# Francis-Fan-create/SCaSML_GP

Hardware: AMD Instinct MI355X
Metric: Euler-Maruyama path-steps/sec + L2 rel-error, Grad_Dependent_Nonlinear d=100 n=3 (higher is better)
Workload: dtype f32

## Files before the change

### include/scasml_hip.h

```cpp
#ifndef SCASML_HIP_H
#define SCASML_HIP_H

#include <stddef.h>
#include <stdint.h>

#ifdef __cplusplus
extern "C" {
#endif

#define SCASML_ABI_VERSION 7
#define SCASML_MAX_LEVEL 5
#define SCASML_MAX_Q 6
#define SCASML_MAX_DIM 252
#define SCASML_GP_TILE 32
#define SCASML_NORMAL_TABLE_ROWS 768

enum { SCASML_ERR_ARG = -1, SCASML_ERR_UNSUPPORTED = -2, SCASML_ERR_HIP = -3 };

enum { SCASML_EQ_GRAD_DEPENDENT_NONLINEAR = 0, SCASML_EQ_CUBIC_REACTION_DIFFUSION = 1, SCASML_EQ_QUADRATIC_GRADIENT_REACTION_DIFFUSION = 2 };

typedef struct {
    int32_t d;
    int32_t eq_id;
    float T;
// ... 138 lines not shown
                              const int32_t *idx_h, int32_t round16, const float *points, int64_t n_inf, int32_t kp, float *grad, void *stream);

int64_t scasml_gp_compat_model_floats(int32_t d, int32_t n_pad);
int scasml_gp_compat_pack_mfma(int32_t d, float a, const float *x_dom, int32_t n_dom, const float *x_bdy, int32_t n_bdy,
                               const double *rv, const int32_t *idx_h, float *model_out, void *stream);
int scasml_gp_eval_compat_sites(int32_t d, float a, float sigma_eq, float mu_eq, int32_t eq_id, const float *model, int32_t n_dom,
                                int32_t n_bdy, const int32_t *idx_h, int32_t round16, float x_bound, const float *points, int64_t n_inf,
                                int64_t rows_per_site, const uint8_t *site_kinds, float *out4, float *lap, void *stream);
int scasml_gp_eval_compat_site_list(int32_t d, float a, float sigma_eq, float mu_eq, int32_t eq_id, const float *model, int32_t n_dom,
                                    int32_t n_bdy, const int32_t *idx_h, int32_t round16, float x_bound, const float *points, int64_t n_inf,
                                    int64_t rows_per_site, const uint8_t *site_kinds, const int32_t *site_order, int32_t n_listed,
                                    float *out4, float *lap, void *stream);

int scasml_gp_cross_rows(int32_t d, double a, const float *x_dom, int32_t n_dom, const float *x_bdy, int32_t n_bdy, const int32_t *idx_h,
                         int32_t round16, int32_t surrogate, int32_t op, const float *x_inf, int64_t n_inf, int64_t ld_inf, double *out,
                         int64_t ld, void *stream);

#define SCASML_DIST_BLOCK 256
int scasml_gp_gram_rows(int32_t d, double a, const float *x_dom, int32_t n_dom, const float *x_bdy, int32_t n_bdy,
                        int64_t row0, int32_t nrows, int64_t ncols, double *out, int64_t ld, void *stream);
int scasml_gp_gram_compat_rows(int32_t d, double a, const float *x_dom, int32_t n_dom, const float *x_bdy, int32_t n_bdy, const int32_t *idx_h,
                               int32_t round16, int64_t row0, int32_t nrows, int64_t ncols, double *out, int64_t ld, void *stream);
int scasml_gemm_nt_sub(double *C, int64_t ldc, int64_t rows, int64_t cols, const double *A, int64_t lda, const double *B,
                       int64_t ldb, int64_t K, int64_t tri_row0, int64_t tri_stride, int64_t tri_col0, void *stream);
int scasml_trsm_right_lt(const double *L, int64_t ldl, int64_t nb, double *X, int64_t ldx, int64_t rows, void *stream);
int scasml_gemv_sub(const double *A, int64_t lda, int64_t rows, int64_t cols, const double *x, double *y, int trans, void *stream);
int64_t scasml_gemv_t_ordered_scratch(int64_t rows, int64_t cols);
int scasml_gemv_t_sub_ordered(const double *A, int64_t lda, int64_t rows, int64_t cols, const double *x, double *y, double *scratch,
                              int64_t scratch_elems, void *stream);
int scasml_gemv_sub_tri(const double *A, int64_t lda, int64_t rows, int64_t cols, const double *x, double *y, int64_t tri_row0, int64_t tri_stride, void *stream);
int scasml_gemv_t_sub_ordered_tri(const double *A, int64_t lda, int64_t rows, int64_t cols, const double *x, double *y, double *scratch,
                                  int64_t scratch_elems, int64_t tri_row0, int64_t tri_stride, void *stream);

#ifdef __cplusplus
}
#endif
#endif
```

### scasml_gp_amd/_build.py

```python
import os
import subprocess
from concurrent.futures import ThreadPoolExecutor

HERE = os.path.dirname(os.path.abspath(__file__))
ROOT = os.path.dirname(HERE)
CSRC = os.path.join(HERE, "csrc")
LIBDIR = os.path.join(HERE, "lib")
LIB = os.path.join(LIBDIR, "libscasml_hip.so")
SOURCES = ["plan_host.cpp", "picard_tree_jax_deep.hip", "picard_tree.hip", "picard_tree_jax.hip", "gp_eval.hip", "gp_eval_bf16.hip", "gp_train.hip", "gp_compat.hip", "gp_eval_compat_mfma.hip", "dist_linalg.hip"]
FLAGS = ["--offload-arch=gfx950", "-O3", "-std=c++17", "-ffp-contract=off", "-fno-slp-vectorize", "-fPIC", "-I" + os.path.join(ROOT, "include")]


def _stale(target, deps):
    if not os.path.exists(target):
        return True
    t = os.path.getmtime(target)
    return any(os.path.getmtime(d) > t for d in deps)


def build_library(force=False, verbose=False):
    hipcc = os.environ.get("HIPCC", "/opt/rocm/bin/hipcc")
    os.makedirs(LIBDIR, exist_ok=True)
    headers = [os.path.join(CSRC, f) for f in os.listdir(CSRC) if f.endswith(".hpp")]
    headers.append(os.path.join(ROOT, "include", "scasml_hip.h"))
    objs, jobs = [], []
    for src in SOURCES:
        s = os.path.join(CSRC, src)
        o = os.path.join(LIBDIR, os.path.splitext(src)[0] + ".o")
        objs.append(o)
        if force or _stale(o, [s] + headers):
            flags = FLAGS if src.endswith(".hip") else [f for f in FLAGS if not f.startswith("--offload-arch")] + ["-x", "c++"]
            jobs.append([hipcc] + flags + ["-c", s, "-o", o])

    def run(cmd):
        if verbose:
            print(" ".join(cmd), flush=True)
        r = subprocess.run(cmd, capture_output=True, text=True)
        if r.returncode != 0:
            raise RuntimeError("hipcc failed:\n" + " ".join(cmd) + "\n" + r.stdout + r.stderr)

    with ThreadPoolExecutor(max_workers=min(8, os.cpu_count() or 4)) as ex:
        list(ex.map(run, jobs))
# ... 8 lines not shown
```

### scasml_gp_amd/_lib.py

```python
import ctypes as C
import os

MAX_LEVEL = 5
MAX_Q = 6
MAX_DIM = 252
GP_TILE = 32
DIST_BLOCK = 256
ABI_VERSION = 7

MODE_MLP, MODE_GENERATE, MODE_ACCUMULATE = 0, 1, 2
RNG_COMPAT_CRN = 1
RNG_COMPAT_F16 = 2
RNG_JAX_STREAM = 4
EQ_GRAD_DEPENDENT_NONLINEAR = 0
EQ_CUBIC_REACTION_DIFFUSION = 1
EQ_QUADRATIC_GRADIENT_REACTION_DIFFUSION = 2


class Problem(C.Structure):
    _fields_ = [("d", C.c_int32), ("eq_id", C.c_int32), ("T", C.c_float), ("mu", C.c_float),
                ("sigma", C.c_float), ("clip", C.c_float)]


class Rng(C.Structure):
    _fields_ = [("seed", C.c_uint64), ("stream", C.c_uint32), ("root0", C.c_uint32),
                ("rank", C.c_int32), ("world", C.c_int32), ("flags", C.c_uint32), ("reserved", C.c_uint32),
                ("unit_owner", C.c_void_p), ("jax_keys", C.c_void_p)]


class Term(C.Structure):
    _fields_ = [("q", C.c_int32), ("mc", C.c_int32), ("sites_l", C.c_int32), ("sites_lm1", C.c_int32),
                ("dfrac", C.c_float * MAX_Q), ("cfrac", C.c_float * MAX_Q),
                ("wfrac", C.c_float * MAX_Q), ("dplus", C.c_float * MAX_Q)]


class Plan(C.Structure):
    _fields_ = [("variant", C.c_int32), ("n", C.c_int32), ("mg", C.c_int32 * (MAX_LEVEL + 1)),
                ("sites", C.c_int32 * (MAX_LEVEL + 1)), ("term", (Term * MAX_LEVEL) * (MAX_LEVEL + 1))]


class GpModel(C.Structure):
    _fields_ = [("d", C.c_int32), ("n_dom", C.c_int32), ("n_bdy", C.c_int32), ("n_pad", C.c_int32),
                ("kp", C.c_int32), ("split", C.c_int32), ("a", C.c_float), ("sigma_eq", C.c_float),
                ("mu_eq", C.c_float), ("eq_id", C.c_int32),
                ("colloc", C.c_void_p), ("colloc_frag", C.c_void_p), ("colloc_bf16", C.c_void_p), ("colloc_is_f16", C.c_int32),
                ("coef", C.c_void_p), ("x_bound", C.c_float), ("reserved", C.c_int32)]


_STRUCTS = (Problem, Rng, Term, Plan, GpModel)
_LIB = None
LIB_PATH = os.environ.get("SCASML_HIP_LIB") or os.path.join(os.path.dirname(os.path.abspath(__file__)), "lib", "libscasml_hip.so")

SIGNATURES = {
    "scasml_abi_version": (C.c_int, []),
    "scasml_last_error": (C.c_char_p, []),
    "scasml_sizeof": (C.c_size_t, [C.c_int]),
    "scasml_points_per_root": (C.c_int64, [C.POINTER(Plan)]),
    "scasml_point_stride": (C.c_int32, [C.c_int32]),
    "scasml_picard_tree": (C.c_int, [C.POINTER(Problem), C.POINTER(Plan), C.c_int, C.c_void_p, C.c_int64, C.c_int64, Rng,
                                     C.c_void_p, C.c_void_p, C.c_void_p, C.c_void_p, C.c_void_p]),
    "scasml_clip": (C.c_int, [C.c_void_p, C.c_int64, C.c_float, C.c_void_p]),
    "scasml_clip_round16": (C.c_int, [C.c_void_p, C.c_int64, C.c_float, C.c_int32, C.c_void_p]),
    "scasml_debug_normals": (C.c_int, [Rng, C.c_uint32, C.c_int32, C.c_int64, C.c_void_p, C.c_void_p]),
    "scasml_debug_jax_normals": (C.c_int, [C.c_uint32, C.c_uint32, C.c_uint64, C.c_int64, C.c_void_p, C.c_void_p]),
    "scasml_debug_transform": (C.c_int, [C.c_uint32, C.c_int64, C.c_void_p, C.c_void_p]),
    "scasml_normal_table_rows": (C.c_int32, []),
    "scasml_normal_table": (C.c_int, [C.c_void_p, C.c_int32]),
    "scasml_gp_plane_halfwords": (C.c_int64, [C.c_int32, C.c_int32]),
    "scasml_gp_coef_floats": (C.c_int64, [C.c_int32]),
    "scasml_gp_pack": (C.c_int, [C.c_int32, C.c_float, C.c_float, C.c_void_p, C.c_int32, C.c_void_p, C.c_int32, C.c_void_p,
                                 C.c_void_p, C.c_void_p, C.c_void_p, C.c_void_p, C.c_void_p]),
    "scasml_gp_eval": (C.c_int, [C.POINTER(GpModel), C.c_void_p, C.c_int64, C.c_void_p, C.c_void_p, C.c_void_p]),
    "scasml_gp_eval_sites": (C.c_int, [C.POINTER(GpModel), C.c_void_p, C.c_int64, C.c_int64, C.c_void_p, C.c_void_p, C.c_void_p]),
    "scasml_plan_site_kinds": (C.c_int, [C.POINTER(Plan), C.c_int32, C.c_int32, C.c_void_p, C.c_void_p]),
    "scasml_plan_deal_units": (C.c_int32, [C.POINTER(Plan), C.c_int32, C.c_void_p, C.c_void_p, C.c_int32, C.c_void_p]),
    "scasml_tile_order_blocks": (C.c_int64, [C.c_int64, C.c_int64, C.c_int32]),
    "scasml_tile_order": (C.c_int, [C.c_int64, C.c_int64, C.c_int64, C.c_int32, C.POINTER(C.c_int64), C.POINTER(C.c_int64)]),
    "scasml_gp_gradient": (C.c_int, [C.POINTER(GpModel), C.c_void_p, C.c_int64, C.c_void_p, C.c_void_p]),
    "scasml_gp_gram": (C.c_int, [C.c_int32, C.c_double, C.c_void_p, C.c_int32, C.c_void_p, C.c_int32, C.c_void_p, C.c_void_p]),
    "scasml_gp_newton_b": (C.c_int, [C.c_int32, C.c_int32, C.c_double, C.c_double, C.c_void_p, C.c_void_p, C.c_int32, C.c_int32, C.c_void_p, C.c_void_p]),
# ... 8 lines not shown
    "scasml_gp_eval_compat": (C.c_int, [C.c_int32, C.c_double, C.c_double, C.c_double, C.c_int32, C.c_void_p, C.c_int32, C.c_int32, C.c_int64, C.c_void_p,
                                        C.c_void_p, C.c_int32, C.c_void_p, C.c_int64, C.c_int32, C.c_void_p, C.c_void_p, C.c_void_p]),
    "scasml_gp_gradient_compat": (C.c_int, [C.c_int32, C.c_double, C.c_void_p, C.c_int32, C.c_int32, C.c_int64, C.c_void_p, C.c_void_p, C.c_int32,
                                            C.c_void_p, C.c_int64, C.c_int32, C.c_void_p, C.c_void_p]),
    "scasml_gp_compat_model_floats": (C.c_int64, [C.c_int32, C.c_int32]),
    "scasml_gp_compat_pack_mfma": (C.c_int, [C.c_int32, C.c_float, C.c_void_p, C.c_int32, C.c_void_p, C.c_int32, C.c_void_p, C.c_void_p,
                                             C.c_void_p, C.c_void_p]),
    "scasml_gp_eval_compat_sites": (C.c_int, [C.c_int32, C.c_float, C.c_float, C.c_float, C.c_int32, C.c_void_p, C.c_int32, C.c_int32, C.c_void_p,
                                              C.c_int32, C.c_float, C.c_void_p, C.c_int64, C.c_int64, C.c_void_p, C.c_void_p, C.c_void_p, C.c_void_p]),
    "scasml_gp_eval_compat_site_list": (C.c_int, [C.c_int32, C.c_float, C.c_float, C.c_float, C.c_int32, C.c_void_p, C.c_int32, C.c_int32, C.c_void_p,
                                                  C.c_int32, C.c_float, C.c_void_p, C.c_int64, C.c_int64, C.c_void_p, C.c_void_p, C.c_int32, C.c_void_p,
                                                  C.c_void_p, C.c_void_p]),
    "scasml_gp_cross_rows": (C.c_int, [C.c_int32, C.c_double, C.c_void_p, C.c_int32, C.c_void_p, C.c_int32, C.c_void_p, C.c_int32, C.c_int32, C.c_int32,
                                       C.c_void_p, C.c_int64, C.c_int64, C.c_void_p, C.c_int64, C.c_void_p]),
    "scasml_gp_gram_rows": (C.c_int, [C.c_int32, C.c_double, C.c_void_p, C.c_int32, C.c_void_p, C.c_int32, C.c_int64, C.c_int32, C.c_int64,
                                      C.c_void_p, C.c_int64, C.c_void_p]),
    "scasml_gp_gram_compat_rows": (C.c_int, [C.c_int32, C.c_double, C.c_void_p, C.c_int32, C.c_void_p, C.c_int32, C.c_void_p, C.c_int32, C.c_int64,
                                             C.c_int32, C.c_int64, C.c_void_p, C.c_int64, C.c_void_p]),
    "scasml_gemm_nt_sub": (C.c_int, [C.c_void_p, C.c_int64, C.c_int64, C.c_int64, C.c_void_p, C.c_int64, C.c_void_p, C.c_int64, C.c_int64,
                                     C.c_int64, C.c_int64, C.c_int64, C.c_void_p]),
    "scasml_gp_newton_jv": (C.c_int, [C.c_int32, C.c_int32, C.c_double, C.c_double, C.c_void_p, C.c_void_p, C.c_int32, C.c_int32, C.c_void_p, C.c_void_p]),
    "scasml_gp_newton_jtv": (C.c_int, [C.c_int32, C.c_int32, C.c_double, C.c_double, C.c_void_p, C.c_void_p, C.c_void_p, C.c_void_p, C.c_double,
                                       C.c_int32, C.c_int32, C.c_void_p, C.c_void_p]),
    "scasml_trsm_right_lt": (C.c_int, [C.c_void_p, C.c_int64, C.c_int64, C.c_void_p, C.c_int64, C.c_int64, C.c_void_p]),
    "scasml_gemv_sub": (C.c_int, [C.c_void_p, C.c_int64, C.c_int64, C.c_int64, C.c_void_p, C.c_void_p, C.c_int, C.c_void_p]),
    "scasml_gemv_t_ordered_scratch": (C.c_int64, [C.c_int64, C.c_int64]),
    "scasml_gemv_t_sub_ordered": (C.c_int, [C.c_void_p, C.c_int64, C.c_int64, C.c_int64, C.c_void_p, C.c_void_p, C.c_void_p, C.c_int64, C.c_void_p]),
    "scasml_gemv_sub_tri": (C.c_int, [C.c_void_p, C.c_int64, C.c_int64, C.c_int64, C.c_void_p, C.c_void_p, C.c_int64, C.c_int64, C.c_void_p]),
    "scasml_gemv_t_sub_ordered_tri": (C.c_int, [C.c_void_p, C.c_int64, C.c_int64, C.c_int64, C.c_void_p, C.c_void_p, C.c_void_p, C.c_int64, C.c_int64, C.c_int64,
                                                C.c_void_p]),
    "scasml_cholesky": (C.c_int, [C.c_void_p, C.c_int64, C.c_double, C.c_void_p, C.c_void_p]),
    "scasml_cholesky_inverse": (C.c_int, [C.c_void_p, C.c_int64, C.c_void_p, C.c_void_p]),
    "scasml_trsm_lower": (C.c_int, [C.c_void_p, C.c_int64, C.c_void_p, C.c_int64, C.c_int, C.c_void_p]),
}


class ScasmlError(RuntimeError):
    pass


def load():
    global _LIB
    if _LIB is not None:
        return _LIB
    import torch
    if not os.path.exists(LIB_PATH):
        raise ScasmlError(
            "libscasml_hip.so is not built (%s missing). Build it with "
            "`python -c 'import __graft_entry__ as g; g.build()'` or `python -m scasml_gp_amd._build`; "
            "scasml_gp_amd has no CPU fallback." % LIB_PATH)
    lib = C.CDLL(LIB_PATH)
    for name, (res, args) in SIGNATURES.items():
        fn = getattr(lib, name)
        fn.restype, fn.argtypes = res, args
    if lib.scasml_abi_version() != ABI_VERSION:
        raise ScasmlError("libscasml_hip.so ABI %d != binding ABI %d" % (lib.scasml_abi_version(), ABI_VERSION))
    for which, st in enumerate(_STRUCTS):
        if lib.scasml_sizeof(which) != C.sizeof(st):
            raise ScasmlError("struct %s: library says %d bytes, binding %d" % (st.__name__, lib.scasml_sizeof(which), C.sizeof(st)))
    _LIB = lib
    return lib


def check(rc, what):
    if rc != 0:
        raise ScasmlError("%s failed (%d): %s" % (what, rc, load().scasml_last_error().decode()))
# ... 17 lines not shown
```

### scasml_gp_amd/csrc/picard_tree.hpp

```cpp
#pragma once
#include <string.h>
#include "common.hpp"
#include "equations.hpp"
#include "philox_normal.hpp"

namespace scasml {

struct TreeArgs {
    scasml_plan plan;
    const float *x_t;
    float *points;
    const float4 *gpv;
    float *out_uz;
    float *out_uhat;
    int64_t B;
    int64_t Bs;
    int64_t ppr;
    uint32_t k0, k1, stream, root0;
    int32_t rank, world;
    const uint8_t *owner;
    int32_t crn;
    int32_t f16;
    const uint32_t *jk;
    int32_t d, G, logG, kp;
    float T, mu, sigma, clip;
};

__device__ __forceinline__ float4 f4(float v) { return make_float4(v, v, v, v); }
__device__ __forceinline__ float4 fma4(float s, float4 a, float4 b) {
    return make_float4(fmaf(s, a.x, b.x), fmaf(s, a.y, b.y), fmaf(s, a.z, b.z), fmaf(s, a.w, b.w));
}
__device__ __forceinline__ float4 add4(float4 a, float s) { return make_float4(a.x + s, a.y + s, a.z + s, a.w + s); }
__device__ __forceinline__ float4 f4_scale(float4 a, float s) { return make_float4(a.x * s, a.y * s, a.z * s, a.w * s); }
__device__ __forceinline__ float4 mul4(float4 a, float4 b) { return make_float4(a.x * b.x, a.y * b.y, a.z * b.z, a.w * b.w); }
__device__ __forceinline__ float clip1(float v, float c) { return v < -c ? -c : (v > c ? c : v); }
__device__ __forceinline__ float r16(float v) { return (float)(_Float16)v; }
__device__ __forceinline__ float rcp_fast(float v) { return __builtin_amdgcn_rcpf(v); }
__device__ __forceinline__ float sqrt_fast(float v) { return __builtin_amdgcn_sqrtf(v); }
__device__ __forceinline__ float exp_fast(float v) { return __builtin_amdgcn_exp2f(v * 1.44269504088896341f); }
// ... 104 lines not shown
    __device__ __forceinline__ float4 normals(uint32_t site) const {
        return mul4(normal4(gl, site, root, a.stream, a.k0, a.k1), mask);
    }
    __device__ __forceinline__ float4 normals_jax(uint32_t kslot, uint64_t row, uint32_t width, uint32_t m) const {
        const uint32_t k0 = a.jk[2 * kslot], k1 = a.jk[2 * kslot + 1];
        const uint64_t first = (row * width + m) * (uint64_t)a.d + 4u * gl;
        float4 v;
        v.x = mask.x != 0.0f ? jax_normal_f16(k0, k1, first + 0) : 0.0f;
        v.y = mask.y != 0.0f ? jax_normal_f16(k0, k1, first + 1) : 0.0f;
        v.z = mask.z != 0.0f ? jax_normal_f16(k0, k1, first + 2) : 0.0f;
        v.w = mask.w != 0.0f ? jax_normal_f16(k0, k1, first + 3) : 0.0f;
        return v;
    }
    template <int N>
    __device__ __forceinline__ uint32_t nsplits() const {
        if constexpr (N <= 0) {
            return 0u;
        } else {
            return nsplits_from<N, 0>();
        }
    }
    template <int N, int L>
    __device__ __forceinline__ uint32_t nsplits_from() const {
        if constexpr (L >= N) {
            return 0u;
        } else {
            const uint32_t per = 1u + nsplits<L>() + nsplits<L - 1>();
            return (uint32_t)a.plan.term[N][L].q * per + nsplits_from<N, L + 1>();
        }
    }
    __device__ __forceinline__ void emit_point(float4 X, float t, uint32_t site) const {
        if (!row_lane) return;
        float4 *base = reinterpret_cast<float4 *>(a.points + (int64_t)site * a.Bs * a.kp);
        base[row_off4] = fma4(t, tmask, mul4(X, mask));
    }
    __device__ __forceinline__ float4 gp_at(uint32_t site) const { return (a.gpv + (int64_t)site * a.Bs)[gp_off]; }
    __device__ __forceinline__ float4 load_point(uint32_t site) const {
        const float4 *base = reinterpret_cast<const float4 *>(a.points + (int64_t)site * a.Bs * a.kp);
        return base[row_off4];
    }
    __device__ __forceinline__ bool mine_at(int un) const {
        return a.owner ? (int)a.owner[un] == a.rank : (un % a.world) == a.rank;
    }
    __device__ __forceinline__ bool owned(bool top) {
        if (!top || a.world == 1) return true;
        const bool mine = mine_at(unit);
        ++unit;
        return mine;
    }

    __device__ __forceinline__ float g_terminal(float4 XT, float u_hat) const {
        float g = EqDef<EQ>::G(dim_sum(EqDef<EQ>::phi(XT)), a.T);
        if (a.f16) g = r16(g);
        if constexpr (MODE == SCASML_MODE_ACCUMULATE) {
            g -= u_hat;
            if (a.f16) g = r16(g);
        }
        return g;
    }
    __device__ __forceinline__ float f_eval(float uc, float4 zc, float4 gp) const {
        const float sz = dim_sum(zc);
        const float fd = (float)a.d;
        if constexpr (EqDef<EQ>::kGradSquare) {
            static_assert(MODE != SCASML_MODE_ACCUMULATE, "an f of |z|^2 needs the surrogate's full gradient per site: not in the fused evaluation");
            const float v = EqDef<EQ>::f2(uc, sz, dim_sum(mul4(zc, zc)), a.sigma, fd);
            return a.f16 ? r16(v) : v;
        } else if constexpr (MODE == SCASML_MODE_ACCUMULATE) {
            const float sg = a.sigma * gp.y;
            const float v1 = EqDef<EQ>::f(uc + gp.x, sg + sz, a.sigma, fd), v2 = EqDef<EQ>::f(gp.x, sg, a.sigma, fd);
            return a.f16 ? r16(r16(v1) - r16(v2)) : v1 - v2;
        } else {
            const float v = EqDef<EQ>::f(uc, sz, a.sigma, fd);
// ... 283 lines not shown
```

### scasml_gp_amd/models/GP.py

```python
import ctypes as C
import os

import numpy as np

from .. import _lib


def _round_up(v, m):
    return (v + m - 1) // m * m


class GP(object):

    def __init__(self, equation, compat="reference", laplacian_idx="partitionable", f16_graph=False):
        if compat == "exact":
            compat = None
        self.eval_geometry = compat == "reference-geometry"
        if self.eval_geometry:
            compat = "reference"
        if compat not in (None, "reference"):
            raise ValueError("compat must be 'reference', 'reference-geometry' or None")
        if compat == "reference" and equation.n_input - 1 < 5:
            raise ValueError("compat='reference' draws five distinct Hutchinson indices from d = %d < 5 coordinates (the reference's "
                             "random.choice(..., replace=False) fails there too); use compat=None" % (equation.n_input - 1))
# ... 100 lines not shown
        lib = _lib.load()
        if self.right_vector is None:
            raise _lib.ScasmlError("GP is not trained: call GPsolver(x_domain, x_boundary) first")
        if self.compat == "reference":
            a = 1.0 / float(self.sigma) ** 2
            xb = x_bound if x_bound > 0 else 2.0
            if self.compat_eval == "mfma" and self._compat_model is not None and 0.7213 * a * xb * xb * (self.d + 1) <= 3.0e4:
                if order is not None and kinds is not None and rows_per_site % 32 == 0 and n_rows % rows_per_site == 0:
                    _lib.check(lib.scasml_gp_eval_compat_site_list(
                        self.d, a, float(self.equation.sigma()), float(self.equation.mu()), int(self.equation.eq_id), _lib.ptr(self._compat_model),
                        self.N_domain, self.N_boundary, self.laplacian_idx.ctypes.data_as(C.c_void_p), int(self.eval_round16), float(x_bound), _lib.ptr(pts),
                        n_rows, rows_per_site, _lib.ptr(kinds), _lib.ptr(order), int(order.numel()), _lib.ptr(out4), None, _lib.stream_ptr()),
                        "gp_eval_compat_site_list")
                    return
                _lib.check(lib.scasml_gp_eval_compat_sites(
                    self.d, a, float(self.equation.sigma()), float(self.equation.mu()), int(self.equation.eq_id), _lib.ptr(self._compat_model),
                    self.N_domain, self.N_boundary, self.laplacian_idx.ctypes.data_as(C.c_void_p), int(self.eval_round16), float(x_bound), _lib.ptr(pts), n_rows,
                    rows_per_site if kinds is not None else 0, _lib.ptr(kinds) if kinds is not None else None, _lib.ptr(out4), None,
                    _lib.stream_ptr()), "gp_eval_compat_sites")
                return
            N = self.N_domain + self.N_boundary
            _lib.check(lib.scasml_gp_eval_compat(self.d, a, float(self.equation.sigma()),
                                                 float(self.equation.mu()), int(self.equation.eq_id), _lib.ptr(self._colloc_t), self.N_domain, self.N_boundary, N, _lib.ptr(self._rv_dev),
                                                 self.laplacian_idx.ctypes.data_as(C.c_void_p), int(self.eval_round16) & 3, _lib.ptr(pts), n_rows,
                                                 pts.shape[1], _lib.ptr(out4), None, _lib.stream_ptr()), "gp_eval_compat")
            return
        model = self._device_model(x_bound)
        if kinds is None:
            _lib.check(lib.scasml_gp_eval(C.byref(model), _lib.ptr(pts), n_rows, _lib.ptr(out4), None, _lib.stream_ptr()), "gp_eval")
        else:
            _lib.check(lib.scasml_gp_eval_sites(C.byref(model), _lib.ptr(pts), n_rows, rows_per_site, _lib.ptr(kinds),
                                                _lib.ptr(out4), _lib.stream_ptr()), "gp_eval")

    def _predict_device(self, x_dev):
        pts, _, hb, f16 = self._points_device(x_dev)
        return self._eval_device(pts, hb, f16)[:, 0:1]

    def kernel_phi_phi(self, x_t_domain, x_t_boundary):
        torch = _lib.require_gpu()
        lib = _lib.load()
        xd = torch.from_numpy(np.ascontiguousarray(np.asarray(x_t_domain), dtype=np.float32)).cuda()
        xb = torch.from_numpy(np.ascontiguousarray(np.asarray(x_t_boundary), dtype=np.float32)).cuda()
        self.N_domain, self.N_boundary = xd.shape[0], xb.shape[0]
        self.phi_dim = M = 4 * self.N_domain + self.N_boundary
        self.x_t_domain, self.x_t_boundary = np.asarray(x_t_domain), np.asarray(x_t_boundary)
        self._xd, self._xb = xd, xb
        s = _lib.stream_ptr()
        K = torch.empty((M, M), dtype=torch.float64, device="cuda")
        if self.compat == "reference":
            colloc_f16 = bool((xd.half().float() == xd).all()) and bool((xb.half().float() == xb).all())
            gram_bits = 1 | ((4 | self._f16_extra) if (self.f16_graph and colloc_f16) else 0)
            self._stage("gram", lambda: _lib.check(lib.scasml_gp_gram_compat(
                self.d, 1.0 / float(self.sigma) ** 2, _lib.ptr(xd), self.N_domain, _lib.ptr(xb), self.N_boundary,
                self.laplacian_idx.ctypes.data_as(C.c_void_p), gram_bits, _lib.ptr(K), s), "gp_gram_compat"))
        else:
            self._stage("gram", lambda: _lib.check(lib.scasml_gp_gram(
                self.d, 1.0 / float(self.sigma) ** 2, _lib.ptr(xd), self.N_domain, _lib.ptr(xb), self.N_boundary, _lib.ptr(K), s), "gp_gram"))
        Mp = _round_up(M, 32)
        L = torch.eye(Mp, dtype=torch.float64, device="cuda")
        L[:M, :M] = K
        info = torch.zeros(1, dtype=torch.int32, device="cuda")
        self._stage("cholesky", lambda: _lib.check(lib.scasml_cholesky(_lib.ptr(L), Mp, float(self.nugget), _lib.ptr(info), s), "cholesky"))
        if int(info.item()) != 0 or bool(torch.isnan(L).any()):
            raise ValueError("Cholesky decomposition resulted in NaN values.")
        self._L_pad = L
        self.cholesky_phi_phi_perturb = L[:M, :M]
# ... 374 lines not shown
```

### scasml_gp_amd/solvers/_picard.py

```python
import ctypes as C
import weakref

import numpy as np

from .. import _lib, tables

POINT_BUFFER_BYTES = 24 << 30


def _as_device(x_t, torch):
    if isinstance(x_t, torch.Tensor):
        return x_t.to(device="cuda", dtype=torch.float32).contiguous(), False, None
    arr = np.ascontiguousarray(np.asarray(x_t), dtype=np.float32)
    return torch.from_numpy(arr).cuda(), True, (float(np.abs(arr).max()) if arr.size else 0.0)


class PicardEngine:
    def __init__(self, equation, variant, gp=None, seed=0, compat_crn=False, compat_f16=False, compat_rng=None, reference_mode=False):
        if reference_mode:
            compat_rng, compat_f16 = "jax", True
        if getattr(equation, "eq_id", None) is None:
            raise NotImplementedError("no HIP kernels for equation %s (eq_id unset)" % type(equation).__name__)
        if getattr(equation, "surrogate_free_only", False) and (gp is not None or reference_mode or compat_rng == "jax"):
            raise NotImplementedError("equation %s has an f of |z|^2: its kernels are the surrogate-free Picard tree on the Philox stream (MLP, MLP_full_history); "
                                      "ScaSML would need the surrogate's full gradient at every tree site" % type(equation).__name__)
        self.equation = equation
        self.variant = variant
        self.gp = gp
        self.seed = int(seed)
        self.compat_crn = bool(compat_crn)
        self.compat_f16 = bool(compat_f16)
        if compat_rng not in (None, "jax"):
            raise ValueError("compat_rng must be None or 'jax'")
        self.compat_rng = compat_rng
        self.jax_key = (0, 0)
        self.jax_splits = 0
        self.calls = 0
        self.profile = False
        self._events = []
        self._plans = {}
        self._kinds = {}
        self._owners = {}
        self._work = {}
        self._bound_cache = None

    def __getstate__(self):
        st = dict(self.__dict__)
        st["_plans"], st["_events"], st["_kinds"], st["_owners"], st["_work"], st["_bound_cache"] = {}, [], {}, {}, {}, None
        return st

    def _timed(self, name, fn):
        if not self.profile:
            return fn()
        torch = _lib.require_gpu()
        e0, e1 = torch.cuda.Event(enable_timing=True), torch.cuda.Event(enable_timing=True)
        e0.record()
        rc = fn()
        e1.record()
        self._events.append((name, e0, e1))
        return rc

    def collect_kernel_ms(self):
        torch = _lib.require_gpu()
        torch.cuda.synchronize()
        acc = {}
        for name, e0, e1 in self._events:
            acc.setdefault(name, []).append(e0.elapsed_time(e1))
        self._events = []
        return {k: sum(v) / len(v) for k, v in acc.items()}

    def plan(self, n, par):
        key = (n, par)
        if key not in self._plans:
            self._plans[key] = tables.build_plan(self.variant, n, par, float(self.equation.T),
                                                 stale_delta_t=self.gp is None)
        return self._plans[key]

    def unit_owners(self, n, par, world):
        key = (n, par, world)
        if key not in self._owners:
            torch = _lib.require_gpu()
            host, load = deal_units(self.plan(n, par), world, site_cost(self.gp))
            self._owners[key] = (host, torch.from_numpy(host).cuda(), load)
        return self._owners[key]

    def site_kinds(self, n, par, rank=0, world=1):
        key = (n, par, rank, world)
        if key not in self._kinds:
            torch = _lib.require_gpu()
            plan = self.plan(n, par)
            ppr = int(_lib.load().scasml_points_per_root(C.byref(plan)))
            host = np.zeros(ppr, dtype=np.uint8)
            owner = self.unit_owners(n, par, world)[0].ctypes.data_as(C.c_void_p) if world > 1 and n > 0 else None
            _lib.check(_lib.load().scasml_plan_site_kinds(C.byref(plan), rank, world, owner, host.ctypes.data_as(C.c_void_p)), "plan_site_kinds")
            self._kinds[key] = torch.from_numpy(host).cuda()
        return self._kinds[key]

    def site_order(self, n, par, rank=0, world=1):
        key = ("order", n, par, rank, world)
        if key not in self._kinds:
            torch = _lib.require_gpu()
# ... 25 lines not shown
        torch = _lib.require_gpu()
        lib = _lib.load()
        x, was_numpy, x_max = _as_device(x_t, torch)
        d = self.equation.n_input - 1
        if x.dim() != 2 or x.shape[1] != d + 1:
            raise ValueError("x_t must have shape (batch, %d), got %s" % (d + 1, tuple(x.shape)))
        B = x.shape[0]
        plan, prob = self.plan(n, par), self.problem()
        if self.gp is not None and float(getattr(self.gp, "T", self.equation.T)) != float(self.equation.T):
            raise _lib.ScasmlError("the surrogate was built for terminal time T = %g, the equation now has T = %g: refit or reload the GP"
                                   % (float(self.gp.T), float(self.equation.T)))
        flags = (_lib.RNG_COMPAT_CRN if self.compat_crn else 0) | (_lib.RNG_COMPAT_F16 if self.compat_f16 else 0)
        owner = self.unit_owners(n, par, world)[1].data_ptr() if world > 1 and n > 0 else None
        jax_keys, jax_next = None, None
        if self.compat_rng == "jax" and n > 0:
            if n > _lib.MAX_LEVEL:
                raise _lib.ScasmlError("picard_tree: level n=%d outside 1..%d" % (n, _lib.MAX_LEVEL))
            keys, jax_next = self._jax_keys(plan)
            jax_keys = keys.data_ptr()
            flags |= _lib.RNG_JAX_STREAM
        rng = _lib.Rng(self.seed, self.calls if stream_id is None else stream_id, root0, rank, world, flags, 0, owner, jax_keys)
        if stream_id is None:
            self.calls += 1
        out = torch.empty((B, d + 1), dtype=torch.float32, device="cuda")
        s = _lib.stream_ptr()
        if self.gp is None:
            _lib.check(self._timed("picard_mlp", lambda: lib.scasml_picard_tree(
                C.byref(prob), C.byref(plan), _lib.MODE_MLP, _lib.ptr(x), B, 0, rng, None, None, _lib.ptr(out), None, s)), "picard_tree")
            self._jax_commit(jax_next, stream_id)
            return out, None, was_numpy
        uhat = torch.empty((B,), dtype=torch.float32, device="cuda")
        ppr = int(lib.scasml_points_per_root(C.byref(plan)))
        kp = int(lib.scasml_point_stride(d))
        chunk = max(1, min(B, POINT_BUFFER_BYTES // (ppr * kp * 4)))
        stride = (chunk + 31) // 32 * 32
        pts, vals = self._buffers(stride * ppr, kp)
        kinds = self.site_kinds(n, par, rank, world) if n > 0 else None
        order = self.site_order(n, par, rank, world) if n > 0 else None
        x_bound = self.path_bound(self._root_bound(x, x_max, x is x_t) if B else None, plan)
        for b0 in range(0, B, chunk):
            nb = min(chunk, B - b0)
            rng_c = _lib.Rng(rng.seed, rng.stream, root0 + b0, rank, world, flags, 0, owner, jax_keys)
            xc = x[b0:b0 + nb]
            if n > 0:
                ob, ub = out[b0:b0 + nb], uhat[b0:b0 + nb]
                _lib.check(self._timed("picard_generate", lambda: lib.scasml_picard_tree(
                    C.byref(prob), C.byref(plan), _lib.MODE_GENERATE, _lib.ptr(xc), nb, stride, rng_c,
                    _lib.ptr(pts), None, None, None, s)), "picard_tree(generate)")
                self._timed("gp_eval", lambda: self.gp._eval_rows(pts, stride * ppr, stride, kinds, vals, x_bound=x_bound, order=order))
                _lib.check(self._timed("picard_accumulate", lambda: lib.scasml_picard_tree(
                    C.byref(prob), C.byref(plan), _lib.MODE_ACCUMULATE, _lib.ptr(xc), nb, stride, rng_c,
                    _lib.ptr(pts), _lib.ptr(vals), _lib.ptr(ob), _lib.ptr(ub), s)), "picard_tree(accumulate)")
            else:
                out[b0:b0 + nb].zero_()
                uhat[b0:b0 + nb] = self.gp._predict_device(xc)[:, 0]
        self._jax_commit(jax_next, stream_id)
        return out, uhat, was_numpy

    def _root_bound(self, x, x_max, own):
        if x_max is not None:
            return x_max
        if not own:
            return float(x.abs().max())
        holder = x._base if x._base is not None else x
        key = (x.data_ptr(), tuple(x.shape), x._version)
        c = self._bound_cache
        if c is None or c[0]() is not holder or c[1] != key:
            self._bound_cache = c = (weakref.ref(holder), key, float(x.abs().max()))
        return c[2]

    def _jax_keys(self, plan):
        from .. import threefry
        torch = _lib.require_gpu()
        q = [[int(plan.term[level][l].q) for l in range(level)] for level in range(plan.n + 1)]
        words, key_after = threefry.solver_key_words(q, plan.n, self.jax_key, quadrature=self.variant == "quad")
        self._work["jax_keys"] = torch.from_numpy(words.view(np.int32).reshape(-1).copy()).cuda()
        return self._work["jax_keys"], (key_after, len(words) - 1)

    def _jax_commit(self, jax_next, stream_id):
        if jax_next is not None and stream_id is None:
            self.jax_key, self.jax_splits = jax_next[0], self.jax_splits + jax_next[1]

    def _buffers(self, rows, kp):
        torch = _lib.require_gpu()
        have = self._work.get("pts")
        if have is None or have.shape[0] < rows or have.shape[1] != kp:
            self._work.pop("pts", None)
            self._work.pop("vals", None)
            self._work["pts"] = torch.zeros((rows, kp), dtype=torch.float32, device="cuda")
            self._work["vals"] = torch.zeros((rows, 4), dtype=torch.float32, device="cuda")
        return self._work["pts"][:rows], self._work["vals"][:rows]

    def finalize_partials(self, summed):
        lib = _lib.load()
        round16 = 1 if (self.compat_f16 and not (self.variant == "fh" and self.gp is not None)) else 0
        _lib.check(lib.scasml_clip_round16(_lib.ptr(summed), summed.numel(), self.problem().clip, round16, _lib.stream_ptr()), "clip")
        return summed

    def evaluation_increment(self, n, par):
        return tables.reference_evaluation_count(self.variant, n, par, self.gp is not None, float(self.equation.T))


SITE_COST = {"reference": (1.0, 0.62, 0.50, 0.04),
             "reference-geometry": (1.0, 0.62, 0.50, 0.06),
             "documented": (1.0, 0.75, 0.50, 0.10),
             None: (1.0, 1.0, 1.0, 0.5)}


def site_cost(gp):
    if gp is None:
        return SITE_COST[None]
    if gp.compat == "reference":
        return SITE_COST["reference-geometry" if getattr(gp, "eval_geometry", False) else "reference"]
    return SITE_COST["documented"]


def deal_units(plan, world, cost=None):
    lib = _lib.load()
    n = plan.n
    units = int(plan.mg[n]) + sum(int(plan.term[n][l].mc) * int(plan.term[n][l].q) * (2 if l else 1) for l in range(n))
    owner = np.zeros(max(units, 1), dtype=np.uint8)
    load = np.zeros(world, dtype=np.float64)
    w = np.ascontiguousarray(cost, dtype=np.float64) if cost is not None else None
    if w is not None and w.shape != (4,):
        raise ValueError("site costs: four numbers (level-0 site, level l > 0 site, terminal site, replayed step)")
    got = lib.scasml_plan_deal_units(C.byref(plan), world, w.ctypes.data_as(C.c_void_p) if w is not None else None,
                                     owner.ctypes.data_as(C.c_void_p), units, load.ctypes.data_as(C.c_void_p))
    if got != units:
        raise _lib.ScasmlError("plan_deal_units failed (%d): %s" % (got, lib.scasml_last_error().decode()))
    return owner[:units].copy(), load


def deliver(t, was_numpy):
# ... 2 lines not shown
```

Measured before the change: 506.9 million.

## Add two-stream chunked pipeline for generate/eval/accumulate and nontemporal point I/O

```diff
diff --git a/include/scasml_hip.h b/include/scasml_hip.h
--- a/include/scasml_hip.h
+++ b/include/scasml_hip.h
@@ -194,6 +194,27 @@
 int scasml_gemv_t_sub_ordered_tri(const double *A, int64_t lda, int64_t rows, int64_t cols, const double *x, double *y, double *scratch,
                                   int64_t scratch_elems, int64_t tri_row0, int64_t tri_stride, void *stream);
 
+typedef struct scasml_pipeline_state scasml_pipeline;
+enum { SCASML_PIPE_EVAL_SITES = 0, SCASML_PIPE_EVAL_COMPAT_SITE_LIST = 1 };
+typedef struct {
+    int32_t kind;
+    int32_t n_listed;
+    const scasml_gp_model *gp_h;
+    int32_t d, eq_id, n_dom, n_bdy, round16, reserved;
+    float a, sigma_eq, mu_eq, x_bound;
+    const float *model;
+    const int32_t *idx_h;
+    const int32_t *site_order;
+} scasml_pipe_eval;
+scasml_pipeline *scasml_pipeline_create(void);
+void scasml_pipeline_destroy(scasml_pipeline *p);
+int64_t scasml_pipeline_chunk_roots(int64_t B, int32_t chunks);
+int64_t scasml_pipeline_ring_rows(const scasml_plan *plan_h, int64_t B, int32_t chunks);
+int scasml_picard_solve_pipelined(scasml_pipeline *p, const scasml_problem *prob_h, const scasml_plan *plan_h, const float *x_t, int64_t B,
+                                  int32_t chunks, scasml_rng rng, const uint8_t *site_kinds, const scasml_pipe_eval *eval_h, float *points,
+                                  float *gp_vals, float *out_uz, float *out_uhat, int32_t timed, void *stream);
+int scasml_pipeline_pass_ms(scasml_pipeline *p, float *ms_h, int32_t capacity);
+
 #ifdef __cplusplus
 }
 #endif
diff --git a/scasml_gp_amd/_build.py b/scasml_gp_amd/_build.py
--- a/scasml_gp_amd/_build.py
+++ b/scasml_gp_amd/_build.py
@@ -7,7 +7,7 @@
 CSRC = os.path.join(HERE, "csrc")
 LIBDIR = os.path.join(HERE, "lib")
 LIB = os.path.join(LIBDIR, "libscasml_hip.so")
-SOURCES = ["plan_host.cpp", "picard_tree_jax_deep.hip", "picard_tree.hip", "picard_tree_jax.hip", "gp_eval.hip", "gp_eval_bf16.hip", "gp_train.hip", "gp_compat.hip", "gp_eval_compat_mfma.hip", "dist_linalg.hip"]
+SOURCES = ["plan_host.cpp", "picard_tree_jax_deep.hip", "picard_tree.hip", "picard_tree_jax.hip", "picard_pipeline.hip", "gp_eval.hip", "gp_eval_bf16.hip", "gp_train.hip", "gp_compat.hip", "gp_eval_compat_mfma.hip", "dist_linalg.hip"]
 FLAGS = ["--offload-arch=gfx950", "-O3", "-std=c++17", "-ffp-contract=off", "-fno-slp-vectorize", "-fPIC", "-I" + os.path.join(ROOT, "include")]
 
 
diff --git a/scasml_gp_amd/_lib.py b/scasml_gp_amd/_lib.py
--- a/scasml_gp_amd/_lib.py
+++ b/scasml_gp_amd/_lib.py
@@ -46,6 +46,15 @@
                 ("colloc", C.c_void_p), ("colloc_frag", C.c_void_p), ("colloc_bf16", C.c_void_p), ("colloc_is_f16", C.c_int32),
                 ("coef", C.c_void_p), ("x_bound", C.c_float), ("reserved", C.c_int32)]
 
+
+class PipeEval(C.Structure):
+    _fields_ = [("kind", C.c_int32), ("n_listed", C.c_int32), ("gp_h", C.POINTER(GpModel)),
+                ("d", C.c_int32), ("eq_id", C.c_int32), ("n_dom", C.c_int32), ("n_bdy", C.c_int32), ("round16", C.c_int32), ("reserved", C.c_int32),
+                ("a", C.c_float), ("sigma_eq", C.c_float), ("mu_eq", C.c_float), ("x_bound", C.c_float),
+                ("model", C.c_void_p), ("idx_h", C.c_void_p), ("site_order", C.c_void_p)]
+
+
+PIPE_EVAL_SITES, PIPE_EVAL_COMPAT_SITE_LIST = 0, 1
 
 _STRUCTS = (Problem, Rng, Term, Plan, GpModel)
 _LIB = None
@@ -120,6 +129,13 @@
     "scasml_cholesky": (C.c_int, [C.c_void_p, C.c_int64, C.c_double, C.c_void_p, C.c_void_p]),
     "scasml_cholesky_inverse": (C.c_int, [C.c_void_p, C.c_int64, C.c_void_p, C.c_void_p]),
     "scasml_trsm_lower": (C.c_int, [C.c_void_p, C.c_int64, C.c_void_p, C.c_int64, C.c_int, C.c_void_p]),
+    "scasml_pipeline_create": (C.c_void_p, []),
+    "scasml_pipeline_destroy": (None, [C.c_void_p]),
+    "scasml_pipeline_chunk_roots": (C.c_int64, [C.c_int64, C.c_int32]),
+    "scasml_pipeline_ring_rows": (C.c_int64, [C.POINTER(Plan), C.c_int64, C.c_int32]),
+    "scasml_picard_solve_pipelined": (C.c_int, [C.c_void_p, C.POINTER(Problem), C.POINTER(Plan), C.c_void_p, C.c_int64, C.c_int32, Rng, C.c_void_p,
+                                                C.POINTER(PipeEval), C.c_void_p, C.c_void_p, C.c_void_p, C.c_void_p, C.c_int32, C.c_void_p]),
+    "scasml_pipeline_pass_ms": (C.c_int, [C.c_void_p, C.c_void_p, C.c_int32]),
 }
 
 
diff --git a/scasml_gp_amd/csrc/picard_pipeline.hip b/scasml_gp_amd/csrc/picard_pipeline.hip
--- /dev/null
+++ b/scasml_gp_amd/csrc/picard_pipeline.hip
@@ -0,0 +1,219 @@
+
+#include <hip/hip_runtime.h>
+
+#include <vector>
+
+#include "common.hpp"
+
+struct scasml_pipeline_state {
+    int device = -1;
+    hipStream_t eval = nullptr;
+    hipStream_t tree = nullptr;
+    hipEvent_t start = nullptr, done_tree = nullptr, done_eval = nullptr;
+    std::vector<hipEvent_t> generated, evaluated;
+    std::vector<hipEvent_t> timing_pool;
+    struct Timed { std::vector<hipEvent_t> ev; int chunks; };
+    std::vector<Timed> pending;
+};
+
+namespace scasml {
+namespace {
+
+int hip_fail(const char *what, hipError_t e) { return fail(SCASML_ERR_HIP, "pipeline: %s: %s", what, hipGetErrorString(e)); }
+
+#define PIPE_HIP(call, what)                              \
+    do {                                                  \
+        const hipError_t e_ = (call);                     \
+        if (e_ != hipSuccess) return hip_fail(what, e_);  \
+    } while (0)
+
+int grow_events(std::vector<hipEvent_t> &v, size_t n, unsigned flags) {
+    while (v.size() < n) {
+        hipEvent_t e;
+        PIPE_HIP(hipEventCreateWithFlags(&e, flags), "hipEventCreateWithFlags");
+        v.push_back(e);
+    }
+    return 0;
+}
+
+int take_timing(scasml_pipeline *p, std::vector<hipEvent_t> &out, size_t n) {
+    out.clear();
+    while (out.size() < n) {
+        if (p->timing_pool.empty()) {
+            hipEvent_t e;
+            PIPE_HIP(hipEventCreateWithFlags(&e, hipEventDefault), "hipEventCreateWithFlags");
+            p->timing_pool.push_back(e);
+        }
+        out.push_back(p->timing_pool.back());
+        p->timing_pool.pop_back();
+    }
+    return 0;
+}
+
+int run_eval(const scasml_pipe_eval &ev, const float *points, int64_t rows, int64_t rows_per_site, const uint8_t *kinds, float *vals,
+             hipStream_t s) {
+    if (ev.kind == SCASML_PIPE_EVAL_SITES) return scasml_gp_eval_sites(ev.gp_h, points, rows, rows_per_site, kinds, vals, s);
+    return scasml_gp_eval_compat_site_list(ev.d, ev.a, ev.sigma_eq, ev.mu_eq, ev.eq_id, ev.model, ev.n_dom, ev.n_bdy, ev.idx_h, ev.round16,
+                                           ev.x_bound, points, rows, rows_per_site, kinds, ev.site_order, ev.n_listed, vals, nullptr, s);
+}
+
+}
+}
+
+using namespace scasml;
+
+extern "C" scasml_pipeline *scasml_pipeline_create(void) {
+    auto *p = new scasml_pipeline_state();
+    hipError_t e = hipGetDevice(&p->device);
+    if (e == hipSuccess) e = hipStreamCreateWithFlags(&p->eval, hipStreamNonBlocking);
+    if (e == hipSuccess) e = hipStreamCreateWithFlags(&p->tree, hipStreamNonBlocking);
+    if (e == hipSuccess) e = hipEventCreateWithFlags(&p->start, hipEventDisableTiming);
+    if (e == hipSuccess) e = hipEventCreateWithFlags(&p->done_tree, hipEventDisableTiming);
+    if (e == hipSuccess) e = hipEventCreateWithFlags(&p->done_eval, hipEventDisableTiming);
+    if (e != hipSuccess) {
+        hip_fail("create", e);
+        scasml_pipeline_destroy(p);
+        return nullptr;
+    }
+    return p;
+}
+
+extern "C" void scasml_pipeline_destroy(scasml_pipeline *p) {
+    if (!p) return;
+    for (auto &t : p->pending)
+        for (hipEvent_t e : t.ev) (void)hipEventDestroy(e);
+    for (auto *v : {&p->generated, &p->evaluated, &p->timing_pool})
+        for (hipEvent_t e : *v) (void)hipEventDestroy(e);
+    if (p->start) (void)hipEventDestroy(p->start);
+    if (p->done_tree) (void)hipEventDestroy(p->done_tree);
+    if (p->done_eval) (void)hipEventDestroy(p->done_eval);
+    if (p->eval) (void)hipStreamDestroy(p->eval);
+    if (p->tree) (void)hipStreamDestroy(p->tree);
+    delete p;
+}
+
+extern "C" int64_t scasml_pipeline_chunk_roots(int64_t B, int32_t chunks) {
+    if (B < 1 || chunks < 1) return -1;
+    const int64_t per = (B + chunks - 1) / chunks;
+    return (per + SCASML_GP_TILE - 1) / SCASML_GP_TILE * SCASML_GP_TILE;
+}
+
+extern "C" int64_t scasml_pipeline_ring_rows(const scasml_plan *plan_h, int64_t B, int32_t chunks) {
+    const int64_t ppr = scasml_points_per_root(plan_h), chunk = scasml_pipeline_chunk_roots(B, chunks);
+    if (ppr < 1 || chunk < 1) return -1;
+    const int64_t run = (B + chunk - 1) / chunk;
+    return (run < 2 ? run : 2) * ppr * chunk;
+}
+
+extern "C" int scasml_picard_solve_pipelined(scasml_pipeline *p, const scasml_problem *prob_h, const scasml_plan *plan_h, const float *x_t,
+                                             int64_t B, int32_t chunks, scasml_rng rng, const uint8_t *site_kinds,
+                                             const scasml_pipe_eval *eval_h, float *points, float *gp_vals, float *out_uz, float *out_uhat,
+                                             int32_t timed, void *stream) {
+    if (!p || !prob_h || !plan_h || !eval_h) return fail(SCASML_ERR_ARG, "picard_solve_pipelined: null argument");
+    if (B < 0 || chunks < 1) return fail(SCASML_ERR_ARG, "picard_solve_pipelined: B = %lld, chunks = %d", (long long)B, chunks);
+    if (B == 0) return 0;
+    if (plan_h->n < 1 || plan_h->n > SCASML_MAX_LEVEL)
+        return fail(SCASML_ERR_UNSUPPORTED, "picard_solve_pipelined: level n=%d outside 1..%d", plan_h->n, SCASML_MAX_LEVEL);
+    if (!x_t || !points || !gp_vals || !out_uz || !site_kinds) return fail(SCASML_ERR_ARG, "picard_solve_pipelined: null buffer");
+    if (eval_h->kind == SCASML_PIPE_EVAL_SITES ? !eval_h->gp_h
+                                               : (eval_h->kind != SCASML_PIPE_EVAL_COMPAT_SITE_LIST || !eval_h->site_order || eval_h->n_listed < 0))
+        return fail(SCASML_ERR_ARG, "picard_solve_pipelined: bad evaluation (kind %d)", eval_h->kind);
+    if (prob_h->d < 1 || prob_h->d > SCASML_MAX_DIM) return fail(SCASML_ERR_UNSUPPORTED, "picard_solve_pipelined: d=%d", prob_h->d);
+    int dev = -1;
+    PIPE_HIP(hipGetDevice(&dev), "hipGetDevice");
+    if (dev != p->device) return fail(SCASML_ERR_ARG, "picard_solve_pipelined: pipeline made on device %d, current device %d", p->device, dev);
+
+    const int64_t chunk = scasml_pipeline_chunk_roots(B, chunks);
+    const int nc = (int)((B + chunk - 1) / chunk);
+    const int64_t ppr = scasml_points_per_root(plan_h), rows = ppr * chunk;
+    const int64_t kp = scasml_point_stride(prob_h->d), d1 = prob_h->d + 1;
+    if (grow_events(p->generated, nc, hipEventDisableTiming) || grow_events(p->evaluated, nc, hipEventDisableTiming))
+        return SCASML_ERR_HIP;
+    scasml_pipeline_state::Timed tm{{}, nc};
+    if (timed && take_timing(p, tm.ev, 6 * (size_t)nc)) return SCASML_ERR_HIP;
+    auto mark = [&](int i, int pass, int end, hipStream_t s) -> hipError_t {
+        return timed ? hipEventRecord(tm.ev[6 * i + 2 * pass + end], s) : hipSuccess;
+    };
+    auto slot_pts = [&](int i) { return points + (int64_t)(i % 2) * rows * kp; };
+    auto slot_vals = [&](int i) { return gp_vals + (int64_t)(i % 2) * rows * 4; };
+    auto tree = [&](int i, int mode) -> int {
+        const int64_t b0 = (int64_t)i * chunk, nb = (B - b0 < chunk) ? B - b0 : chunk;
+        scasml_rng r = rng;
+        r.root0 = rng.root0 + (uint32_t)b0;
+        const int pass = mode == SCASML_MODE_GENERATE ? 0 : 2;
+        PIPE_HIP(mark(i, pass, 0, p->tree), "hipEventRecord");
+        const int rc = mode == SCASML_MODE_GENERATE
+                           ? scasml_picard_tree(prob_h, plan_h, mode, x_t + b0 * d1, nb, chunk, r, slot_pts(i), nullptr, nullptr, nullptr, p->tree)
+                           : scasml_picard_tree(prob_h, plan_h, mode, x_t + b0 * d1, nb, chunk, r, slot_pts(i), slot_vals(i), out_uz + b0 * d1,
+                                                out_uhat ? out_uhat + b0 : nullptr, p->tree);
+        if (rc) return rc;
+        PIPE_HIP(mark(i, pass, 1, p->tree), "hipEventRecord");
+        if (mode == SCASML_MODE_GENERATE) PIPE_HIP(hipEventRecord(p->generated[i], p->tree), "hipEventRecord");
+        return 0;
+    };
+    auto eval = [&](int i) -> int {
+        PIPE_HIP(hipStreamWaitEvent(p->eval, p->generated[i], 0), "hipStreamWaitEvent");
+        PIPE_HIP(mark(i, 1, 0, p->eval), "hipEventRecord");
+        const int rc = run_eval(*eval_h, slot_pts(i), rows, chunk, site_kinds, slot_vals(i), p->eval);
+        if (rc) return rc;
+        PIPE_HIP(mark(i, 1, 1, p->eval), "hipEventRecord");
+        PIPE_HIP(hipEventRecord(p->evaluated[i], p->eval), "hipEventRecord");
+        return 0;
+    };
+    auto accumulate = [&](int i) -> int {
+        PIPE_HIP(hipStreamWaitEvent(p->tree, p->evaluated[i], 0), "hipStreamWaitEvent");
+        return tree(i, SCASML_MODE_ACCUMULATE);
+    };
+
+    int rc = 0;
+    PIPE_HIP(hipEventRecord(p->start, (hipStream_t)stream), "hipEventRecord");
+    PIPE_HIP(hipStreamWaitEvent(p->tree, p->start, 0), "hipStreamWaitEvent");
+    PIPE_HIP(hipStreamWaitEvent(p->eval, p->start, 0), "hipStreamWaitEvent");
+    if ((rc = tree(0, SCASML_MODE_GENERATE)) || (rc = eval(0))) goto end;
+    if (nc > 1 && (rc = tree(1, SCASML_MODE_GENERATE))) goto end;
+    for (int i = 1; i < nc; ++i) {
+        if ((rc = eval(i)) || (rc = accumulate(i - 1))) goto end;
+        if (i + 1 < nc && (rc = tree(i + 1, SCASML_MODE_GENERATE))) goto end;
+    }
+    rc = accumulate(nc - 1);
+end:
+    {
+        const hipError_t e1 = hipEventRecord(p->done_tree, p->tree);
+        const hipError_t e2 = e1 == hipSuccess ? hipStreamWaitEvent((hipStream_t)stream, p->done_tree, 0) : e1;
+        const hipError_t e3 = hipEventRecord(p->done_eval, p->eval);
+        const hipError_t e4 = e3 == hipSuccess ? hipStreamWaitEvent((hipStream_t)stream, p->done_eval, 0) : e3;
+        if (!rc && e2 != hipSuccess) rc = hip_fail("join", e2);
+        if (!rc && e4 != hipSuccess) rc = hip_fail("join", e4);
+    }
+    if (timed) {
+        if (rc) {
+            for (hipEvent_t e : tm.ev) p->timing_pool.push_back(e);
+        } else {
+            p->pending.push_back(std::move(tm));
+        }
+    }
+    return rc;
+}
+
+extern "C" int scasml_pipeline_pass_ms(scasml_pipeline *p, float *ms_h, int32_t capacity) {
+    if (!p || (capacity > 0 && !ms_h) || capacity < 0) return fail(SCASML_ERR_ARG, "pipeline_pass_ms: bad argument");
+    int rc = 0;
+    const int n = (int)p->pending.size();
+    for (int k = 0; k < n; ++k) {
+        auto &t = p->pending[k];
+        float sum[3] = {0.0f, 0.0f, 0.0f};
+        for (int i = 0; i < t.chunks && !rc; ++i)
+            for (int pass = 0; pass < 3 && !rc; ++pass) {
+                float ms = 0.0f;
+                hipError_t e = hipEventSynchronize(t.ev[6 * i + 2 * pass + 1]);
+                if (e == hipSuccess) e = hipEventElapsedTime(&ms, t.ev[6 * i + 2 * pass], t.ev[6 * i + 2 * pass + 1]);
+                if (e != hipSuccess) rc = hip_fail("pass_ms", e);
+                sum[pass] += ms;
+            }
+        if (!rc && k < capacity)
+            for (int pass = 0; pass < 3; ++pass) ms_h[3 * k + pass] = sum[pass];
+        for (hipEvent_t e : t.ev) p->timing_pool.push_back(e);
+    }
+    p->pending.clear();
+    return rc ? rc : n;
+}
diff --git a/scasml_gp_amd/csrc/picard_tree.hpp b/scasml_gp_amd/csrc/picard_tree.hpp
--- a/scasml_gp_amd/csrc/picard_tree.hpp
+++ b/scasml_gp_amd/csrc/picard_tree.hpp
@@ -5,6 +5,8 @@
 #include "philox_normal.hpp"
 
 namespace scasml {
+
+typedef float nt_float4 __attribute__((ext_vector_type(4)));
 
 struct TreeArgs {
     scasml_plan plan;
@@ -175,12 +177,15 @@
     __device__ __forceinline__ void emit_point(float4 X, float t, uint32_t site) const {
         if (!row_lane) return;
         float4 *base = reinterpret_cast<float4 *>(a.points + (int64_t)site * a.Bs * a.kp);
-        base[row_off4] = fma4(t, tmask, mul4(X, mask));
+        const float4 v = fma4(t, tmask, mul4(X, mask));
+        const nt_float4 w = {v.x, v.y, v.z, v.w};
+        __builtin_nontemporal_store(w, reinterpret_cast<nt_float4 *>(base + row_off4));
     }
     __device__ __forceinline__ float4 gp_at(uint32_t site) const { return (a.gpv + (int64_t)site * a.Bs)[gp_off]; }
     __device__ __forceinline__ float4 load_point(uint32_t site) const {
         const float4 *base = reinterpret_cast<const float4 *>(a.points + (int64_t)site * a.Bs * a.kp);
-        return base[row_off4];
+        const nt_float4 w = __builtin_nontemporal_load(reinterpret_cast<const nt_float4 *>(base + row_off4));
+        return make_float4(w.x, w.y, w.z, w.w);
     }
     __device__ __forceinline__ bool mine_at(int un) const {
         return a.owner ? (int)a.owner[un] == a.rank : (un % a.world) == a.rank;
diff --git a/scasml_gp_amd/models/GP.py b/scasml_gp_amd/models/GP.py
--- a/scasml_gp_amd/models/GP.py
+++ b/scasml_gp_amd/models/GP.py
@@ -156,6 +156,27 @@
             _lib.check(lib.scasml_gp_eval_sites(C.byref(model), _lib.ptr(pts), n_rows, rows_per_site, _lib.ptr(kinds),
                                                 _lib.ptr(out4), _lib.stream_ptr()), "gp_eval")
 
+    def _pipe_eval(self, x_bound, order):
+        if self.right_vector is None:
+            raise _lib.ScasmlError("GP is not trained: call GPsolver(x_domain, x_boundary) first")
+        if "_eval_rows" in vars(self):
+            return None
+        ev = _lib.PipeEval()
+        if self.compat == "reference":
+            a = 1.0 / float(self.sigma) ** 2
+            xb = x_bound if x_bound > 0 else 2.0
+            if not (self.compat_eval == "mfma" and self._compat_model is not None and 0.7213 * a * xb * xb * (self.d + 1) <= 3.0e4):
+                return None
+            idx = np.ascontiguousarray(self.laplacian_idx, dtype=np.int32)
+            ev.kind, ev.n_listed, ev.site_order = _lib.PIPE_EVAL_COMPAT_SITE_LIST, int(order.numel()), order.data_ptr()
+            ev.d, ev.eq_id, ev.n_dom, ev.n_bdy, ev.round16 = self.d, int(self.equation.eq_id), self.N_domain, self.N_boundary, int(self.eval_round16)
+            ev.a, ev.sigma_eq, ev.mu_eq, ev.x_bound = a, float(self.equation.sigma()), float(self.equation.mu()), float(x_bound)
+            ev.model, ev.idx_h = self._compat_model.data_ptr(), idx.ctypes.data
+            return ev, (idx, order, self._compat_model)
+        model = self._device_model(x_bound)
+        ev.kind, ev.gp_h = _lib.PIPE_EVAL_SITES, C.pointer(model)
+        return ev, (model,)
+
     def _predict_device(self, x_dev):
         pts, _, hb, f16 = self._points_device(x_dev)
         return self._eval_device(pts, hb, f16)[:, 0:1]
diff --git a/scasml_gp_amd/solvers/_picard.py b/scasml_gp_amd/solvers/_picard.py
--- a/scasml_gp_amd/solvers/_picard.py
+++ b/scasml_gp_amd/solvers/_picard.py
@@ -6,6 +6,7 @@
 from .. import _lib, tables
 
 POINT_BUFFER_BYTES = 24 << 30
+PIPELINE_CHUNKS = 1
 
 
 def _as_device(x_t, torch):
@@ -16,7 +17,8 @@
 
 
 class PicardEngine:
-    def __init__(self, equation, variant, gp=None, seed=0, compat_crn=False, compat_f16=False, compat_rng=None, reference_mode=False):
+    def __init__(self, equation, variant, gp=None, seed=0, compat_crn=False, compat_f16=False, compat_rng=None, reference_mode=False,
+                 pipeline_chunks=None):
         if reference_mode:
             compat_rng, compat_f16 = "jax", True
         if getattr(equation, "eq_id", None) is None:
@@ -43,10 +45,13 @@
         self._owners = {}
         self._work = {}
         self._bound_cache = None
+        self.pipeline_chunks = pipeline_chunks
+        self._pipes = {}
 
     def __getstate__(self):
         st = dict(self.__dict__)
         st["_plans"], st["_events"], st["_kinds"], st["_owners"], st["_work"], st["_bound_cache"] = {}, [], {}, {}, {}, None
+        st["_pipes"] = {}
         return st
 
     def _timed(self, name, fn):
@@ -67,6 +72,10 @@
         for name, e0, e1 in self._events:
             acc.setdefault(name, []).append(e0.elapsed_time(e1))
         self._events = []
+        for pipe in self._pipes.values():
+            for ms in pipe.pass_ms():
+                for name, v in zip(("picard_generate", "gp_eval", "picard_accumulate"), ms):
+                    acc.setdefault(name, []).append(v)
         return {k: sum(v) / len(v) for k, v in acc.items()}
 
     def plan(self, n, par):
@@ -158,12 +167,26 @@
         uhat = torch.empty((B,), dtype=torch.float32, device="cuda")
         ppr = int(lib.scasml_points_per_root(C.byref(plan)))
         kp = int(lib.scasml_point_stride(d))
+        kinds = self.site_kinds(n, par, rank, world) if n > 0 else None
+        order = self.site_order(n, par, rank, world) if n > 0 else None
+        x_bound = self.path_bound(self._root_bound(x, x_max, x is x_t) if B else None, plan)
+        chunks = int(self.pipeline_chunks or PIPELINE_CHUNKS)
+        pipe = self.gp._pipe_eval(x_bound, order) if n > 0 and B > 0 and chunks > 1 else None
+        if pipe is not None:
+            chunks = max(chunks, -(-2 * B * ppr * kp * 4 // POINT_BUFFER_BYTES))
+            pts, vals = self._buffers(int(lib.scasml_pipeline_ring_rows(C.byref(plan), B, chunks)), kp)
+            ev, _keep = pipe
+            timed = self.profile
+            _lib.check(lib.scasml_picard_solve_pipelined(
+                self._pipeline(), C.byref(prob), C.byref(plan), _lib.ptr(x), B, chunks, rng, _lib.ptr(kinds), C.byref(ev), _lib.ptr(pts),
+                _lib.ptr(vals), _lib.ptr(out), _lib.ptr(uhat), 1 if timed else 0, s), "picard_solve_pipelined")
+            if timed:
+                self._pipeline_obj().timed += 1
+            self._jax_commit(jax_next, stream_id)
+            return out, uhat, was_numpy
         chunk = max(1, min(B, POINT_BUFFER_BYTES // (ppr * kp * 4)))
         stride = (chunk + 31) // 32 * 32
         pts, vals = self._buffers(stride * ppr, kp)
-        kinds = self.site_kinds(n, par, rank, world) if n > 0 else None
-        order = self.site_order(n, par, rank, world) if n > 0 else None
-        x_bound = self.path_bound(self._root_bound(x, x_max, x is x_t) if B else None, plan)
         for b0 in range(0, B, chunk):
             nb = min(chunk, B - b0)
             rng_c = _lib.Rng(rng.seed, rng.stream, root0 + b0, rank, world, flags, 0, owner, jax_keys)
@@ -183,6 +206,16 @@
         self._jax_commit(jax_next, stream_id)
         return out, uhat, was_numpy
 
+    def _pipeline_obj(self):
+        torch = _lib.require_gpu()
+        dev = torch.cuda.current_device()
+        if dev not in self._pipes:
+            self._pipes[dev] = _Pipeline()
+        return self._pipes[dev]
+
+    def _pipeline(self):
+        return C.c_void_p(self._pipeline_obj().handle)
+
     def _root_bound(self, x, x_max, own):
         if x_max is not None:
             return x_max
@@ -225,6 +258,31 @@
 
     def evaluation_increment(self, n, par):
         return tables.reference_evaluation_count(self.variant, n, par, self.gp is not None, float(self.equation.T))
+
+
+class _Pipeline:
+
+    def __init__(self):
+        self.lib = _lib.load()
+        self.handle = self.lib.scasml_pipeline_create()
+        if not self.handle:
+            raise _lib.ScasmlError("pipeline_create failed: %s" % self.lib.scasml_last_error().decode())
+        self.timed = 0
+
+    def pass_ms(self):
+        if not self.timed:
+            return []
+        ms = np.zeros((self.timed, 3), dtype=np.float32)
+        got = self.lib.scasml_pipeline_pass_ms(C.c_void_p(self.handle), ms.ctypes.data_as(C.c_void_p), self.timed)
+        self.timed = 0
+        if got < 0:
+            raise _lib.ScasmlError("pipeline_pass_ms failed (%d): %s" % (got, self.lib.scasml_last_error().decode()))
+        return [tuple(float(v) for v in row) for row in ms[:got]]
+
+    def __del__(self):
+        if getattr(self, "handle", None):
+            self.lib.scasml_pipeline_destroy(C.c_void_p(self.handle))
+            self.handle = None
 
 
 SITE_COST = {"reference": (1.0, 0.62, 0.50, 0.04),
```

Result: no change. 507.8 million, median of 6 (+0.2%).
